# lastdancewithyou/multimodal_edema_prediction

Hardware: AMD Instinct MI355X
Metric: multimodal train samples/sec (higher is better)
Workload: dtype bf16

## Files before the change

### multimodal_edema_prediction_amd/csrc/gemm_bf16_v7.hip

```cpp
#include <string.h>

#include <atomic>

#include "common.h"
#include "gemm_tile256.h"
#include "gemm_variants.h"

namespace {

constexpr int SLOT_WORDS = 16;
constexpr int RING_SLOTS = 1024, CAPTURE_SLOTS = 15360;
__device__ unsigned g_v7_slots[(RING_SLOTS + CAPTURE_SLOTS) * SLOT_WORDS];

constexpr int BM = 256;
constexpr int PROW = 144;
constexpr int PATCH = 16 * PROW;
constexpr int MAILBOX = 2 * KBUF + 8 * PATCH;
constexpr int BIASBUF = MAILBOX + 256;
constexpr int TRACEBUF = BIASBUF + 2048;
constexpr int STATBUF = TRACEBUF + 512;
constexpr int CSBUF = STATBUF + 256 * 4 * 2 * 4;
constexpr int LDS_BYTES = CSBUF + 2048;
static_assert(LDS_BYTES <= 160 * 1024, "K buffers + patches + mailbox exceed the LDS");
constexpr int NWG = 256;

#ifdef MEDP_V7_PHASE_TRACE
#define PT(k)                                                          \
    do {                                                               \
        const unsigned now_ = (unsigned)__builtin_readcyclecounter();  \
        pt_acc[k] += now_ - pt_last;                                   \
        pt_last = now_;                                                \
    } while (0)
#else
#define PT(k) do { } while (0)
#endif

template <int TAG, bool FOLD = false>
__global__ __launch_bounds__(512, 2) void gemm_bf16_nt_v7_kernel(const MedpGemmArgs p, unsigned* slot, unsigned long long* trace, const int MB, const int SN) {
    extern __shared__ __attribute__((aligned(16))) char smem[];
    const int tid = threadIdx.x, lane = tid & 63;
    const int wave = __builtin_amdgcn_readfirstlane(tid >> 6);
    const int fr = lane & 15, kq = lane >> 4;
    const int wm = wave >> 2, wn = wave & 3;
    const bf16_t* A = (const bf16_t*)p.A;
    const bf16_t* W = (const bf16_t*)p.W;
    const bf16_t* zero = (const bf16_t*)g_zero16_t256;
    MEDP_PROF_ENTER(p.prof, p.prof_flags);

    const Tile256Map map(p.M, p.N, BM);
    const int ntiles = map.tiles_m * map.tiles_n;
    const int nkt = p.K >> 6;
    const int xcd = blockIdx.x & 7;

    int m0, n0;
    map.origin(blockIdx.x, MB, SN, BM, m0, n0);

    const int srow = tid >> 3, schunk = (tid & 7) ^ (srow & 7);
    const unsigned voff_a = ((unsigned)srow * (unsigned)p.lda + (unsigned)(schunk * 8)) * 2u;
    const unsigned voff_w = ((unsigned)srow * (unsigned)p.ldw + (unsigned)(schunk * 8)) * 2u;
    medp_rsrc_t ra[4], rw[4];
    auto set_m = [&](int mm) {
#pragma unroll
        for (int q = 0; q < 4; ++q) {
            const int rows = mm < 0 ? 0 : min(64, max(0, p.M - mm - q * 64));
            ra[q] = lds_dma_rsrc(A + (size_t)(mm < 0 ? 0 : mm + q * 64) * (size_t)p.lda, (unsigned)__builtin_amdgcn_readfirstlane(rows * p.lda * 2));
        }
    };
    auto set_n = [&](int nn) {
#pragma unroll
        for (int q = 0; q < 4; ++q) {
            const int rows = nn < 0 ? 0 : min(64, max(0, p.N - nn - q * 64));
            rw[q] = lds_dma_rsrc(W + (size_t)(nn < 0 ? 0 : nn + q * 64) * (size_t)p.ldw, (unsigned)__builtin_amdgcn_readfirstlane(rows * p.ldw * 2));
        }
    };
    set_m(m0);
    set_n(n0);
#ifdef MEDP_V7_ABLATE_LOADS
    bool ablate_on = false;
#endif
    auto stage_piece = [&](int k0, int b, int which, int j) {
#ifdef MEDP_V7_ABLATE_LOADS
        if (ablate_on) return;
#endif
        char* dst = piece_dst(smem, b, which, wave, j);
        const int q = (which & 1) * 2 + j;
        if (which < 2) blds16(ra[q], voff_a, (unsigned)k0 * 2u, dst);
        else blds16(rw[q], voff_w, (unsigned)k0 * 2u, dst);
    };
    auto stage_a = [&](int k0, int b, int j) { stage_piece(k0, b, 0, j); stage_piece(k0, b, 1, j); };
    auto stage_w = [&](int k0, int b, int h) { stage_piece(k0, b, 2 + h, 0); stage_piece(k0, b, 2 + h, 1); };
    typedef __attribute__((address_space(3))) volatile int lds_int;
    lds_int* mailbox = (lds_int*)(__attribute__((address_space(3))) char*)(smem + MAILBOX);
    typedef __attribute__((address_space(3))) volatile unsigned long long lds_u64;
    lds_u64* tbuf = (lds_u64*)(__attribute__((address_space(3))) char*)(smem + TRACEBUF);
    int tcount = 0;
    auto stamp = [&](int k, long long tile) {
        if (trace && wave == 0 && tcount < 8) {
            if (k == 0) tbuf[tcount * 5] = (unsigned long long)tile;
            tbuf[tcount * 5 + 1 + k] = wall_clock64();
        }
    };

    f32x4 acc[8][4];

    const int sw = fr & 7;
    const int fa_off = wm * HALF + fr * 128;
    const int fw_off = 2 * HALF + (wn >> 1) * HALF + ((wn & 1) * 64 + fr) * 128;
    const int ch0 = ((0 + kq) ^ sw) << 4, ch1 = ((4 + kq) ^ sw) << 4;

    bf16x8 fa[4][2], fw0a[2][2], fw0b[2][2], fw1[2][2];
    auto read_a = [&](const char* buf, int a) {
#pragma unroll
        for (int i = 0; i < 4; ++i) {
            const char* rp = buf + fa_off + (a * 64 + i * 16) * 128;
            fa[i][0] = *(const bf16x8*)(rp + ch0);
            fa[i][1] = *(const bf16x8*)(rp + ch1);
        }
    };
    auto read_w = [&](const char* buf, int b, bf16x8 (*fw)[2]) {
#pragma unroll
        for (int j = 0; j < 2; ++j) {
            const char* rp = buf + fw_off + (b * 32 + j * 16) * 128;
            fw[j][0] = *(const bf16x8*)(rp + ch0);
            fw[j][1] = *(const bf16x8*)(rp + ch1);
        }
    };
    bool rows_live[2];
    auto mma = [&](int a, int b, const bf16x8 (*fw)[2]) {
        if (!rows_live[a]) return;
#ifdef MEDP_V7_ABLATE_MFMA
#pragma unroll
        for (int i = 0; i < 4; ++i) { asm volatile("" ::"v"(fa[i][0]), "v"(fa[i][1])); }
#pragma unroll
        for (int j = 0; j < 2; ++j) { asm volatile("" ::"v"(fw[j][0]), "v"(fw[j][1])); }
        return;
#endif
        __builtin_amdgcn_s_setprio(1);
#pragma unroll
        for (int kh = 0; kh < 2; ++kh)
#pragma unroll
            for (int i = 0; i < 4; ++i)
#pragma unroll
                for (int j = 0; j < 2; ++j)
                    acc[a * 4 + i][b * 2 + j] = __builtin_amdgcn_mfma_f32_16x16x32_bf16(fw[j][kh], fa[i][kh], acc[a * 4 + i][b * 2 + j], 0, 0, 0);
        __builtin_amdgcn_s_setprio(0);
    };

    unsigned ticket = 0;
    auto draw_ticket = [&]() {
        if (tid == 0) {
            const unsigned one = 1;
            asm volatile("global_atomic_add %0, %1, %2, off sc0" : "=&v"(ticket) : "v"(slot + xcd), "v"(one) : "memory");
        }
    };
    auto post_ticket = [&]() {
        if (wave == 0) {
            const int tn = (int)gridDim.x + 8 * (int)ticket + xcd;
            mailbox[lane] = tn < ntiles ? tn : -1;
        }
    };

    auto stage_bias = [&](int nn, bool live, int which) {
        if (wave == 0) {
            const int nj = nn + lane * 4;
            const float* src = (live && p.bias && nj < p.N) ? p.bias + nj : (const float*)zero;
            glds16(src, smem + BIASBUF + which * 1024);
        }
    };
    int bias_cur = 0;
    const MedpGemmFold& fo = p.fold;
    constexpr bool consumer = FOLD;
    auto opaque = [](int x) { asm volatile("" : "+v"(x)); return x; };
    auto stage_cs = [&](int nn, bool live, int which) {
        if (consumer && wave == 1) {
            const int nj = nn + opaque(lane) * 4;
            const float* src = (live && nj < p.N) ? fo.colsum + nj : (const float*)zero;
            glds16(src, smem + CSBUF + which * 1024);
        }
    };
    auto stage_stats = [&](int mm) {
        if (consumer && wave * 1024 < 256 * fo.stats_tiles * 8)
            glds16((const char*)fo.stats_in + (size_t)mm * fo.stats_tiles * 8 + wave * 1024 + opaque(lane) * 16, smem + STATBUF + wave * 1024);
    };

    stage_bias(n0, true, 0);
    stage_cs(n0, true, 0);
    stage_stats(m0);
    draw_ticket();
    stage_a(0, 0, 0); stage_w(0, 0, 0); stage_w(0, 0, 1); stage_a(0, 0, 1);
    stage_a(64, 1, 0); stage_w(64, 1, 0); stage_w(64, 1, 1);
    __builtin_amdgcn_s_waitcnt(0x0f70);
    asm volatile("" : "+v"(ticket)::"memory");
    post_ticket();
    bool first = true;
#ifdef MEDP_V7_ABLATE_LOADS
    ablate_on = true;
#endif

#ifdef MEDP_V7_PHASE_TRACE
    unsigned pt_acc[17], pt_last = 0;
#pragma unroll
    for (int i = 0; i < 17; ++i) pt_acc[i] = 0;
#endif
    for (;;) {
        MEDP_BAR();
        stamp(0, ((long long)m0 << 32) | (unsigned)n0);
        rows_live[0] = m0 + wm * 128 < p.M;
        rows_live[1] = m0 + wm * 128 + 64 < p.M;
        float z;
        asm volatile("v_mov_b32 %0, 0" : "=v"(z));
#pragma unroll
        for (int i = 0; i < 8; ++i)
#pragma unroll
            for (int j = 0; j < 4; ++j) acc[i][j] = (f32x4){z, z, z, z};
        if (first) read_w(smem, 0, fw0a);
        else stage_stats(m0);
        first = false;
        if (wm == 1) MEDP_BAR();

#ifdef MEDP_V7_PHASE_TRACE
        pt_last = (unsigned)__builtin_readcyclecounter();
#endif
        int t_next = -1, m0n = 0, n0n = 0;
        auto before_p2 = [&](int kt) {
            if (kt == nkt - 2) {
                t_next = __builtin_amdgcn_readfirstlane(mailbox[0]);
                if (t_next >= 0) map.origin(t_next, MB, SN, BM, m0n, n0n);
                set_m(t_next >= 0 ? m0n : -1);
                set_n(t_next >= 0 ? n0n : -1);
            }
        };
        auto clock = [&](int k) { PT(k); };
        auto ktile = [&](int kt, const bf16x8 (*fw0)[2], bf16x8 (*fw0n)[2]) {
            const int k2 = kt + 2 < nkt ? (kt + 2) * 64 : (kt + 2 - nkt) * 64;
            const int k1 = kt + 1 < nkt ? (kt + 1) * 64 : 0;
            const int b2 = kt & 1;
            auto stream_a = [&](int t, int j) { if (t == kt + 1) stage_a(k1, b2 ^ 1, j); else stage_a(k2, b2, j); };
            auto stream_w = [&](int, int h) { stage_w(k2, b2, h); };
            tile256_ktile<true>(smem, kt, fw0, fw0n, fw1, read_a, read_w, mma, stream_a, stream_w, before_p2, clock);
        };
#pragma clang loop unroll(disable)
        for (int kt = 0; kt < nkt; kt += 2) {
            ktile(kt, fw0a, fw0b);
            ktile(kt + 1, fw0b, fw0a);
        }
        if (wm == 0) MEDP_BAR();

        stamp(1, 0);
        draw_ticket();
        stage_bias(n0n, t_next >= 0, bias_cur ^ 1);
        stage_cs(n0n, t_next >= 0, bias_cur ^ 1);

        f32x4 bj[4];
        if constexpr (!FOLD) {
#pragma unroll
            for (int j = 0; j < 4; ++j) bj[j] = *(const f32x4*)(smem + BIASBUF + bias_cur * 1024 + (wn * 64 + j * 16 + kq * 4) * 4);
        }
        char* wl = smem + 2 * KBUF + wave * PATCH;
        const bool full_tile = m0 + BM <= p.M && n0 + BN <= p.N;
        const int prow = lane >> 3, pchunk = lane & 7;
        const int ncol = n0 + wn * 64 + pchunk * 8;
        typedef __attribute__((ext_vector_type(2))) unsigned int u32x2;
        typedef __attribute__((ext_vector_type(4))) unsigned int u32x4;
        const float inv_dim = consumer ? 1.0f / (float)fo.ln_dim : 0.f;
#pragma unroll
        for (int i = 0; i < 8; ++i) {
            float rstd = 1.f, mr = 0.f;
            if constexpr (consumer) {
                const float* sr = (const float*)(smem + STATBUF) + (wm * 128 + i * 16 + opaque(fr)) * fo.stats_tiles * 2;
                float a1 = 0.f, a2 = 0.f;
                for (int t = 0; t < fo.stats_tiles; ++t) {
                    const float2 st = *(const float2*)(sr + 2 * t);
                    a1 += st.x;
                    a2 += st.y;
                }
                const float mean = a1 * inv_dim;
                rstd = rsqrtf(fmaxf(a2 * inv_dim - mean * mean, 0.f) + fo.ln_eps);
                mr = mean * rstd;
            }
#pragma unroll
            for (int j = 0; j < 4; ++j) {
                f32x4 v;
                if constexpr (consumer) {
                    const f32x4 cj = *(const f32x4*)(smem + CSBUF + bias_cur * 1024 + (wn * 64 + j * 16 + kq * 4) * 4);
                    const f32x4 bb = *(const f32x4*)(smem + BIASBUF + bias_cur * 1024 + (wn * 64 + j * 16 + kq * 4) * 4);
                    v = acc[i][j] * rstd - mr * cj + bb;
                } else {
                    v = acc[i][j] + bj[j];
                }
                if (p.act == 1) v = gelu_bf16_4(v);
                *(u32x2*)(wl + fr * PROW + j * 32 + kq * 8) = (u32x2){pack_bf2(v[0], v[1]), pack_bf2(v[2], v[3])};
            }
            MEDP_WAVE_LDS_SYNC();
#pragma unroll
            for (int h = 0; h < 2; ++h) {
                const int row = h * 8 + prow;
                const int m = m0 + wm * 128 + i * 16 + row;
                const u32x4 o = *(const u32x4*)(wl + row * PROW + pchunk * 16);
                if (m < p.M && ncol < p.N) __builtin_nontemporal_store(o, (u32x4*)((bf16_t*)p.C + (size_t)m * p.ldc + ncol));
            }
            MEDP_WAVE_LDS_SYNC();
        }
        stamp(2, 0);
        if (full_tile) __builtin_amdgcn_s_waitcnt(0x4f70);
        else __builtin_amdgcn_s_waitcnt(0x0f70);
        asm volatile("" : "+v"(ticket)::"memory");
        stamp(3, 0);
        ++tcount;
        post_ticket();
        bias_cur ^= 1;
        if (t_next < 0) break;
        m0 = m0n;
        n0 = n0n;
    }
    if (trace && wave == 0) {
        __builtin_amdgcn_s_waitcnt(0xc07f);
        if (lane < 40) trace[(size_t)blockIdx.x * 40 + lane] = lane < tcount * 5 ? tbuf[lane] : 0ull;
    }
#ifdef MEDP_V7_PHASE_TRACE
    if (trace && lane < 16) {
        unsigned v = 0;
#pragma unroll
        for (int i = 0; i < 16; ++i) v = lane == i ? pt_acc[i] : v;
        trace[256 * 40 + ((size_t)blockIdx.x * 8 + wave) * 16 + lane] = v;
    }
#endif
    if (tid == 0) {
        const unsigned left = __hip_atomic_fetch_add(slot + 8, 1u, __ATOMIC_RELAXED, __HIP_MEMORY_SCOPE_AGENT);
        if (left == gridDim.x - 1) {
#pragma unroll
            for (int i = 0; i < 9; ++i) __hip_atomic_store(slot + i, 0u, __ATOMIC_RELAXED, __HIP_MEMORY_SCOPE_AGENT);
        }
    }
    MEDP_PROF_LEAVE(p.prof, p.prof_flags);
}

std::atomic<unsigned> g_ring_next{0}, g_capture_next{0};
std::atomic<int> g_api_cap{0};
unsigned long long* g_trace = nullptr;

unsigned* ticket_block(hipStream_t stream) {
    static unsigned* slots_of[MEDP_MAX_DEVICES] = {};
    int dev = 0;
    (void)hipGetDevice(&dev);
    MEDP_ONCE_PER_DEVICE({
        unsigned* sp = nullptr;
        if (hipGetSymbolAddress((void**)&sp, HIP_SYMBOL(g_v7_slots)) == hipSuccess) slots_of[dev % MEDP_MAX_DEVICES] = sp;
    });
    unsigned* slots = slots_of[dev % MEDP_MAX_DEVICES];
    if (!slots) return nullptr;
    hipStreamCaptureStatus cs = hipStreamCaptureStatusNone;
    hipStreamIsCapturing(stream, &cs);
    unsigned s;
    if (cs == hipStreamCaptureStatusActive) {
        s = g_capture_next.fetch_add(1);
        if (s >= (unsigned)CAPTURE_SLOTS) return nullptr;
        s += RING_SLOTS;
    } else {
        s = g_ring_next.fetch_add(1) % RING_SLOTS;
    }
    return slots + (size_t)s * SLOT_WORDS;
}

template <int TAG, bool FOLD>
int launch_v7(const MedpGemmArgs& a, hipStream_t stream) {
    MEDP_ONCE_PER_DEVICE({
        (void)hipFuncSetAttribute((const void*)gemm_bf16_nt_v7_kernel<TAG, FOLD>, hipFuncAttributeMaxDynamicSharedMemorySize, LDS_BYTES);
    });
    unsigned* slot = ticket_block(stream);
    if (!slot) return -1;
    static const int env_cap = [] { const int v = medp_env_int("MEDP_V7_WGS", NWG); return (v >= 8 && v <= NWG) ? (v & ~7) : NWG; }();
    const int api_cap = g_api_cap.load();
    const int cap = api_cap > 0 ? api_cap : env_cap;
    const int ntiles = ((a.M + BM - 1) / BM) * ((a.N + BN - 1) / BN);
    const int rounds = (ntiles + cap - 1) / cap;
    static const int fewest = medp_env_int("MEDP_V7_FEWEST_WGS", 1);
    const int nwg = fewest ? min(cap, ((ntiles + rounds - 1) / rounds + 7) & ~7) : cap;
    static const int env_mb = medp_env_int("MEDP_V7_BLOCK", 0);
    static const int env_sn = [] { const char* e = getenv("MEDP_V7_BLOCK"); const char* x = e ? strchr(e, 'x') : nullptr; return x ? atoi(x + 1) : 0; }();
    int mb = 8, sn = 4;
    if (env_mb > 0 && env_sn > 0) { mb = env_mb; sn = env_sn; }
    gemm_bf16_nt_v7_kernel<TAG, FOLD><<<nwg, 512, LDS_BYTES, stream>>>(a, slot, g_trace, mb, sn);
    MEDP_LAUNCH_CHECK("medp_gemm_bf16_nt(v7)");
    return 0;
}

}

bool medp_gemm_v7_supports(const MedpGemmArgs& a) {
    return a.out_bf16 && a.residual == nullptr && a.scale == nullptr && a.N % 8 == 0 && a.ldc % 8 == 0 &&
           a.K % 128 == 0 && a.K >= 256 && (long long)a.M * a.lda < (1ll << 31) && (long long)a.N * a.ldw < (1ll << 31) &&
           a.lda < (1 << 24) && a.ldw < (1 << 24);
}

bool medp_gemm_v7_eligible(const MedpGemmArgs& a) {
    const int tiles = ((a.M + BM - 1) / BM) * ((a.N + BN - 1) / BN);
    return tiles > NWG && medp_gemm_v7_supports(a);
}

int medp_gemm_v7_launch(const MedpGemmArgs& a, int tag, void* stream) {
    if (a.fold.stats_in) return launch_v7<1, true>(a, (hipStream_t)stream);
    return tag == 1 ? launch_v7<1, false>(a, (hipStream_t)stream) : launch_v7<0, false>(a, (hipStream_t)stream);
}

unsigned* medp_gemm_ticket_block(void* stream) { return ticket_block((hipStream_t)stream); }

extern "C" int medp_gemm_persistent_cap(int cap) {
    const int v = cap <= 0 ? 0 : (cap < 8 ? 8 : (cap > NWG ? NWG : (cap & ~7)));
    return g_api_cap.exchange(v);
}

extern "C" int medp_dbg_gemm_v7_trace(void* buf) {
    g_trace = (unsigned long long*)buf;
    return 0;
}
```

Baseline: 13460.

## Pipeline full-tile GEMM epilogue and use single buffer resource per operand

Replaces the four per-quarter buffer resource descriptors for A and W with one descriptor per operand and a computed soffset per piece, cutting SGPR use and descriptor setup when tiles change. Adds a software-pipelined epilogue for full, non-folded tiles: while the global stores of one 16-row block are issued, the next block is bias-added, activated, packed and staged through the LDS patch. Bounds checks are dropped on this path, and the activation is a compile-time branch. The supported leading-dimension limit is tightened to keep the larger offsets in 32-bit range.

```diff
diff --git a/multimodal_edema_prediction_amd/csrc/gemm_bf16_v7.hip b/multimodal_edema_prediction_amd/csrc/gemm_bf16_v7.hip
--- a/multimodal_edema_prediction_amd/csrc/gemm_bf16_v7.hip
+++ b/multimodal_edema_prediction_amd/csrc/gemm_bf16_v7.hip
@@ -1,6 +1,7 @@
 #include <string.h>
 
 #include <atomic>
+#include <type_traits>
 
 #include "common.h"
 #include "gemm_tile256.h"
@@ -58,20 +59,15 @@
     const int srow = tid >> 3, schunk = (tid & 7) ^ (srow & 7);
     const unsigned voff_a = ((unsigned)srow * (unsigned)p.lda + (unsigned)(schunk * 8)) * 2u;
     const unsigned voff_w = ((unsigned)srow * (unsigned)p.ldw + (unsigned)(schunk * 8)) * 2u;
-    medp_rsrc_t ra[4], rw[4];
+    const unsigned piece_a = (unsigned)p.lda * 128u, piece_w = (unsigned)p.ldw * 128u;
+    medp_rsrc_t ra, rw;
     auto set_m = [&](int mm) {
-#pragma unroll
-        for (int q = 0; q < 4; ++q) {
-            const int rows = mm < 0 ? 0 : min(64, max(0, p.M - mm - q * 64));
-            ra[q] = lds_dma_rsrc(A + (size_t)(mm < 0 ? 0 : mm + q * 64) * (size_t)p.lda, (unsigned)__builtin_amdgcn_readfirstlane(rows * p.lda * 2));
-        }
+        const int rows = mm < 0 ? 0 : min(BM, max(0, p.M - mm));
+        ra = lds_dma_rsrc(A + (size_t)(mm < 0 ? 0 : mm) * (size_t)p.lda, (unsigned)__builtin_amdgcn_readfirstlane(rows * p.lda) * 2u);
     };
     auto set_n = [&](int nn) {
-#pragma unroll
-        for (int q = 0; q < 4; ++q) {
-            const int rows = nn < 0 ? 0 : min(64, max(0, p.N - nn - q * 64));
-            rw[q] = lds_dma_rsrc(W + (size_t)(nn < 0 ? 0 : nn + q * 64) * (size_t)p.ldw, (unsigned)__builtin_amdgcn_readfirstlane(rows * p.ldw * 2));
-        }
+        const int rows = nn < 0 ? 0 : min(BN, max(0, p.N - nn));
+        rw = lds_dma_rsrc(W + (size_t)(nn < 0 ? 0 : nn) * (size_t)p.ldw, (unsigned)__builtin_amdgcn_readfirstlane(rows * p.ldw) * 2u);
     };
     set_m(m0);
     set_n(n0);
@@ -84,8 +80,8 @@
 #endif
         char* dst = piece_dst(smem, b, which, wave, j);
         const int q = (which & 1) * 2 + j;
-        if (which < 2) blds16(ra[q], voff_a, (unsigned)k0 * 2u, dst);
-        else blds16(rw[q], voff_w, (unsigned)k0 * 2u, dst);
+        if (which < 2) blds16(ra, voff_a, (unsigned)q * piece_a + (unsigned)k0 * 2u, dst);
+        else blds16(rw, voff_w, (unsigned)q * piece_w + (unsigned)k0 * 2u, dst);
     };
     auto stage_a = [&](int k0, int b, int j) { stage_piece(k0, b, 0, j); stage_piece(k0, b, 1, j); };
     auto stage_w = [&](int k0, int b, int h) { stage_piece(k0, b, 2 + h, 0); stage_piece(k0, b, 2 + h, 1); };
@@ -263,43 +259,88 @@
         typedef __attribute__((ext_vector_type(2))) unsigned int u32x2;
         typedef __attribute__((ext_vector_type(4))) unsigned int u32x4;
         const float inv_dim = consumer ? 1.0f / (float)fo.ln_dim : 0.f;
-#pragma unroll
-        for (int i = 0; i < 8; ++i) {
-            float rstd = 1.f, mr = 0.f;
-            if constexpr (consumer) {
-                const float* sr = (const float*)(smem + STATBUF) + (wm * 128 + i * 16 + opaque(fr)) * fo.stats_tiles * 2;
-                float a1 = 0.f, a2 = 0.f;
-                for (int t = 0; t < fo.stats_tiles; ++t) {
-                    const float2 st = *(const float2*)(sr + 2 * t);
-                    a1 += st.x;
-                    a2 += st.y;
+        auto pack_block = [&](int i, auto act, u32x2 (&pk)[4]) {
+#pragma unroll
+            for (int j = 0; j < 4; ++j) {
+                f32x4 v = acc[i][j] + bj[j];
+                if constexpr (decltype(act)::value) v = gelu_bf16_4(v);
+                pk[j] = (u32x2){pack_bf2(v[0], v[1]), pack_bf2(v[2], v[3])};
+            }
+        };
+        auto epilogue_full = [&](auto act) {
+            char* cp = (char*)((bf16_t*)p.C + (size_t)(m0 + wm * 128 + prow) * p.ldc + ncol);
+            const size_t rows8 = (size_t)p.ldc * 16;
+            u32x2 pk[4];
+            u32x4 o[2];
+            auto through_patch = [&]() {
+#pragma unroll
+                for (int j = 0; j < 4; ++j) *(u32x2*)(wl + fr * PROW + j * 32 + kq * 8) = pk[j];
+                MEDP_WAVE_LDS_SYNC();
+#pragma unroll
+                for (int h = 0; h < 2; ++h) o[h] = *(const u32x4*)(wl + (h * 8 + prow) * PROW + pchunk * 16);
+                MEDP_WAVE_LDS_SYNC();
+            };
+            pack_block(0, act, pk);
+            through_patch();
+#pragma unroll
+            for (int i = 0; i < 8; ++i) {
+                __builtin_amdgcn_sched_barrier(0);
+                if (i + 1 < 8) pack_block(i + 1, act, pk);
+                __builtin_amdgcn_sched_barrier(0);
+#pragma unroll
+                for (int h = 0; h < 2; ++h) {
+                    __builtin_nontemporal_store(o[h], (u32x4*)cp);
+                    cp += rows8;
                 }
-                const float mean = a1 * inv_dim;
-                rstd = rsqrtf(fmaxf(a2 * inv_dim - mean * mean, 0.f) + fo.ln_eps);
-                mr = mean * rstd;
+                if (i + 1 < 8) through_patch();
             }
-#pragma unroll
-            for (int j = 0; j < 4; ++j) {
-                f32x4 v;
+        };
+        const bool pipelined = !FOLD && full_tile;
+        if constexpr (!FOLD) {
+            if (full_tile) {
+                if (p.act == 1) epilogue_full(std::true_type{});
+                else epilogue_full(std::false_type{});
+            }
+        }
+        if (!pipelined) {
+#pragma unroll
+            for (int i = 0; i < 8; ++i) {
+                float rstd = 1.f, mr = 0.f;
                 if constexpr (consumer) {
-                    const f32x4 cj = *(const f32x4*)(smem + CSBUF + bias_cur * 1024 + (wn * 64 + j * 16 + kq * 4) * 4);
-                    const f32x4 bb = *(const f32x4*)(smem + BIASBUF + bias_cur * 1024 + (wn * 64 + j * 16 + kq * 4) * 4);
-                    v = acc[i][j] * rstd - mr * cj + bb;
-                } else {
-                    v = acc[i][j] + bj[j];
+                    const float* sr = (const float*)(smem + STATBUF) + (wm * 128 + i * 16 + opaque(fr)) * fo.stats_tiles * 2;
+                    float a1 = 0.f, a2 = 0.f;
+                    for (int t = 0; t < fo.stats_tiles; ++t) {
+                        const float2 st = *(const float2*)(sr + 2 * t);
+                        a1 += st.x;
+                        a2 += st.y;
+                    }
+                    const float mean = a1 * inv_dim;
+                    rstd = rsqrtf(fmaxf(a2 * inv_dim - mean * mean, 0.f) + fo.ln_eps);
+                    mr = mean * rstd;
                 }
-                if (p.act == 1) v = gelu_bf16_4(v);
-                *(u32x2*)(wl + fr * PROW + j * 32 + kq * 8) = (u32x2){pack_bf2(v[0], v[1]), pack_bf2(v[2], v[3])};
+#pragma unroll
+                for (int j = 0; j < 4; ++j) {
+                    f32x4 v;
+                    if constexpr (consumer) {
+                        const f32x4 cj = *(const f32x4*)(smem + CSBUF + bias_cur * 1024 + (wn * 64 + j * 16 + kq * 4) * 4);
+                        const f32x4 bb = *(const f32x4*)(smem + BIASBUF + bias_cur * 1024 + (wn * 64 + j * 16 + kq * 4) * 4);
+                        v = acc[i][j] * rstd - mr * cj + bb;
+                    } else {
+                        v = acc[i][j] + bj[j];
+                    }
+                    if (p.act == 1) v = gelu_bf16_4(v);
+                    *(u32x2*)(wl + fr * PROW + j * 32 + kq * 8) = (u32x2){pack_bf2(v[0], v[1]), pack_bf2(v[2], v[3])};
+                }
+                MEDP_WAVE_LDS_SYNC();
+#pragma unroll
+                for (int h = 0; h < 2; ++h) {
+                    const int row = h * 8 + prow;
+                    const int m = m0 + wm * 128 + i * 16 + row;
+                    const u32x4 o = *(const u32x4*)(wl + row * PROW + pchunk * 16);
+                    if (m < p.M && ncol < p.N) __builtin_nontemporal_store(o, (u32x4*)((bf16_t*)p.C + (size_t)m * p.ldc + ncol));
+                }
+                MEDP_WAVE_LDS_SYNC();
             }
-            MEDP_WAVE_LDS_SYNC();
-#pragma unroll
-            for (int h = 0; h < 2; ++h) {
-                const int row = h * 8 + prow;
-                const int m = m0 + wm * 128 + i * 16 + row;
-                const u32x4 o = *(const u32x4*)(wl + row * PROW + pchunk * 16);
-                if (m < p.M && ncol < p.N) __builtin_nontemporal_store(o, (u32x4*)((bf16_t*)p.C + (size_t)m * p.ldc + ncol));
-            }
-            MEDP_WAVE_LDS_SYNC();
         }
         stamp(2, 0);
         if (full_tile) __builtin_amdgcn_s_waitcnt(0x4f70);
@@ -390,7 +431,7 @@
 bool medp_gemm_v7_supports(const MedpGemmArgs& a) {
     return a.out_bf16 && a.residual == nullptr && a.scale == nullptr && a.N % 8 == 0 && a.ldc % 8 == 0 &&
            a.K % 128 == 0 && a.K >= 256 && (long long)a.M * a.lda < (1ll << 31) && (long long)a.N * a.ldw < (1ll << 31) &&
-           a.lda < (1 << 24) && a.ldw < (1 << 24);
+           a.lda < (1 << 23) && a.ldw < (1 << 23);
 }
 
 bool medp_gemm_v7_eligible(const MedpGemmArgs& a) {
```

Result: faster. 13600, median of 6 (+1.0%).
